# nullmax-vision/SimPB

Measured on AMD Instinct MI355X. Metric: frames/sec (6-cam sample) + MSDeformAttn HBM GB/s, R50 704x256 @1/2/4/8 GPU, higher is better.
Workload: dtype f32

## Files before the change

include/simpb_hip.h:

```cpp
#ifndef SIMPB_HIP_H
#define SIMPB_HIP_H

#ifdef __cplusplus
extern "C" {
#endif

#define SIMPB_OK 0
#define SIMPB_EINVAL 1
#define SIMPB_ELAUNCH 2

#define SIMPB_RECORD3D_WIDTH 15

int simpb_abi_version(void);

const char* simpb_last_error(void);

#define SIMPB_KERNEL_DAF 1
#define SIMPB_KERNEL_MSDA 2
int simpb_timing_enable(int capacity);
int simpb_timing_read(int kernel_id, float* ms_out, int max_n);
void simpb_timing_reset(void);

int simpb_deformable_aggregation_forward(
    float* output, const float* mc_ms_feat, const int* spatial_shape, const int* scale_start_index,
    const float* sample_location, const float* weights,
    int batch_size, int num_cams, int num_feat, int num_embeds, int num_scale,
    int num_anchors, int num_pts, int num_groups, void* stream);

int simpb_dfa_fused_forward(
    float* output, const void* mc_ms_feat, int feat_is_f16, const int* spatial_shape, const int* scale_start_index,
    const float* anchor, const float* learnable, const float* fix_scale, const float* projection_mat, const float* image_wh,
    const float* feat_logits, const float* cam_logits, float* loc_out, float* weights_out, int batch_size, int num_cams,
    int num_feat, int num_embeds, int num_scale, int num_anchors, int num_fix, int num_learn, int num_groups, void* stream);
int simpb_dfa_fused_forward_cams(
    float* output, const void* mc_ms_feat, int feat_is_f16, const int* spatial_shape, const int* scale_start_index,
    const float* anchor, const float* learnable, const float* fix_scale, const float* projection_mat, const float* image_wh,
    const float* feat_logits, const float* cam_logits, float* loc_out, float* weights_out, int batch_size, int num_cams,
    int num_feat, int num_embeds, int num_scale, int num_anchors, int num_fix, int num_learn, int num_groups,
    const unsigned char* cam_valid, void* stream);


int simpb_deformable_aggregation_backward(
    float* grad_mc_ms_feat, float* grad_sampling_location, float* grad_weights, const float* mc_ms_feat,
    const int* spatial_shape, const int* scale_start_index, const float* sample_location, const float* weights,
    const float* grad_output, int batch_size, int num_cams, int num_feat, int num_embeds, int num_scale,
    int num_anchors, int num_pts, int num_groups, void* stream);

int simpb_ms_deform_attn_grouped_forward(
    float* output, const float* value, const long long* spatial_shapes, const long long* level_start,
    const float* sampling_loc, const float* attn_weight, const int* query_cam,
    int batch_size, int num_cams, int num_value, int num_heads, int channels,
    int num_levels, int num_points, int num_query, void* stream);

int simpb_msda_linear_forward(float* agg, int ld_agg, const void* tokens, int tokens_are_f16,
                              const long long* spatial_shapes, const long long* level_start, const float* raw,
                              int ld_raw, const float* ref, int ld_ref, const int* query_cam, const int* m_live,
                              int batch_size, int num_cams, int num_value, int num_heads, int channels,
                              int num_levels, int num_points, int num_query, void* stream);

int simpb_ms_deform_attn_grouped_backward(
    float* grad_value, float* grad_sampling_loc, float* grad_attn_weight, const float* value,
    const long long* spatial_shapes, const long long* level_start, const float* sampling_loc, const float* attn_weight,
    const int* query_cam, const float* grad_output, int batch_size, int num_cams, int num_value, int num_heads,
    int channels, int num_levels, int num_points, int num_query, void* stream);

int simpb_linear_f32(float* y, const float* x, const float* weight, const float* bias, int M, int N, int K,
                     int relu, void* stream);

int simpb_linear_f16x3(float* y, const float* x, const void* weight_hi, const void* weight_lo, const float* bias, int M,
                       int N, int K, void* stream);

int simpb_linear_f16in_split(float* y, const void* x_f16, const void* weight_hi, const void* weight_lo, const float* bias,
                             int M, int N, int K, void* stream);

int simpb_stem_conv7x7_pool_f16(void* out, const void* img_nhwc4, const void* weight_packed, const void* bias,
                                int num_images, int height, int width, int out_channels, void* stream);

int simpb_image_to_nhwc4_f16(void* out, const float* img, long long stride_n, long long stride_c, long long stride_h,
                             long long stride_w, int num_images, int channels, int height, int width, void* stream);

#define SIMPB_PREPROCESS_MAX_TAPS 64
int simpb_preprocess_u8_nhwc4_f16(void* out, const void* src, void* mid, const int* kx, const int* xlo, const int* xn,
                                  const int* ky, const int* ylo, const int* yn, const void* lut, int num_images,
                                  int src_height, int src_width, int out_height, int out_width, int taps_x, int taps_y,
                                  int src_row0, int src_rows, int flip, int swap_rb, void* stream);

int simpb_preprocess_yuv420sp_nhwc4_f16(void* out, const void* src, void* mid, const int* kx, const int* xlo, const int* xn,
                                        const int* ky, const int* ylo, const int* yn, const void* lut, int num_images,
                                        int src_height, int src_width, int out_height, int out_width, int taps_x, int taps_y,
                                        int src_row0, int src_rows, int flip, int swap_rb, int vu_order, int yoff, int iy,
                                        int irv, int igu, int igv, int ibu, void* stream);

#define SIMPB_SURFACE_BGR 0
#define SIMPB_SURFACE_NV12 1
#define SIMPB_SURFACE_NV21 2
#define SIMPB_SURFACE_P010 3
int simpb_preprocess_surface_nhwc4_f16(void* out, const void* src, const void* image_table, void* mid, const int* kx,
                                       const int* xlo, const int* xn, const int* ky, const int* ylo, const int* yn,
                                       const void* lut, int num_images, int src_height, int src_width, int out_height,
                                       int out_width, int taps_x, int taps_y, int src_row0, int src_rows, int flip, int swap_rb,
                                       int format, long long pitch, long long chroma_pitch, long long chroma_offset,
                                       long long image_stride, int yoff, int iy, int irv, int igu, int igv, int ibu,
                                       void* stream);

int simpb_preprocess_mid_pitch(int out_width);

#define SIMPB_GEMM_MAX_SEGS 4
#define SIMPB_GEMM_MAX_JOBS 4
#define SIMPB_GEMM_OUT_F32 0
#define SIMPB_GEMM_OUT_SPLIT_HALFS 1
typedef struct simpb_gemm_job {
  const float* x[SIMPB_GEMM_MAX_SEGS];
  int ldx[SIMPB_GEMM_MAX_SEGS];
  int kseg[SIMPB_GEMM_MAX_SEGS];
  int num_seg;
  int M, N, K;
  const float* w;
  const float* bias;
  float* y;
  const int* m_live;
  int ldw, ldy, relu;
  int out_fmt;
  const int* row_flag;
  const float* bias2;
  const void* w_hi;
  const void* w_lo;
} simpb_gemm_job;
typedef struct simpb_gemm_args {
  int num_jobs;
  int reserved;
  simpb_gemm_job job[SIMPB_GEMM_MAX_JOBS];
} simpb_gemm_args;
int simpb_gemm_f32(const simpb_gemm_args* args, void* stream);

int simpb_layernorm_f32(float* out, int ldo, const float* x0, int ld0, int k0, const float* x1, int ld1, int k1,
                        const float* gamma, const float* beta, int num_rows, const int* m_live, void* stream);

#define SIMPB_MAX_LEVELS 8
int simpb_format_tokens(float* col_feats, const void* const* level_ptrs, const void* const* level_bias,
                        const int* level_hw, int num_levels, int num_images, int channels, int src_is_half, void* stream);

int simpb_bias_act_nhwc_f16(void* y, const void* bias, const void* residual, long long num_pixels, int channels,
                            int relu, void* stream);

int simpb_bias_relu_maxpool_nhwc_f16(void* y, const void* x, const void* bias, int num_images, int in_h, int in_w,
                                     int channels, void* stream);

int simpb_conv1x1_nhwc_f16(void* y, const void* x, const void* weight, const void* bias, const void* residual,
                           int num_images, int in_h, int in_w, int in_channels, int out_channels, int stride, int relu,
                           int residual_upsample2x, const void* input_bias, int variant, void* stream);

int simpb_conv3x3_nhwc_f16(void* y, float* tokens, void* tokens_f16, int tokens_per_cam, int level_start, const void* x,
                           const void* weight, const void* bias, int num_images, int in_h, int in_w, int in_channels,
                           int out_channels, int stride, int relu, int variant, void* stream);

int simpb_conv3x3_choose_variant(long long p_out, int in_channels, int out_channels);

int simpb_conv3x3_group_tokens_f16(int num_levels, float* tokens, void* tokens_f16, int tokens_per_cam, const int* level_start,
                                   const void* const* x, const void* const* weight, const void* const* bias, int num_images,
                                   const int* in_h, const int* in_w, int in_channels, int out_channels, int relu, void* stream);

int simpb_attention_f32(float* out, const float* q, const float* k, const float* v, const int* query_cam,
                        const int* group_start, int batch_size, int num_heads, int head_dim, int num_query,
                        int num_key, int ldq, int ldk, int ldv, int ldo, float scale, void* stream);

int simpb_attention_f32_split(float* out, const float* q, const float* k, const float* v, const int* query_cam,
                              const int* group_start, int batch_size, int num_heads, int head_dim, int num_query,
                              int num_key, int ldq, int ldk, int ldv, int ldo, float scale, void* stream);

int simpb_attention_split_halfs(float* out, const void* q, const void* k, const void* v, const int* query_cam,
                                const int* group_start, int batch_size, int num_heads, int head_dim, int num_query,
                                int num_key, int ldq, int ldk, int ldv, int ldo, void* stream);

#define SIMPB_MLP_MAX_OPS 12
#define SIMPB_MLP_MAX_CHAINS 8
#define SIMPB_MLP_POST_NONE 0
#define SIMPB_MLP_POST_REFINE3D 1
#define SIMPB_MLP_POST_REFINE2D 2
#define SIMPB_MLP_POST_SIGMOID 3
#define SIMPB_MLP_LINEAR 0
#define SIMPB_MLP_LAYERNORM 1
#define SIMPB_MLP_IN_ROWS 0
#define SIMPB_MLP_IN_SINE2D 1
#define SIMPB_MLP_IN_ROWS_LN 2
typedef struct simpb_mlp_op {
  int type, in_dim, out_dim, relu;
  const float* w;
  const float* b;
} simpb_mlp_op;
typedef struct simpb_mlp_chain {
  const float* x;
  const float* x2;
  float* out;
  const float* out_scale;
  int ldx, ldx2, ldo, in_dim, in_mode, n_ops;
  int post, ldres, res_cols, div_rows, div_col0, reserved;
  const float* res;
  const float* div;
  simpb_mlp_op ops[SIMPB_MLP_MAX_OPS];
  const float* ln_w;
  const float* ln_b;
  float* ln_out;
  int ld_ln_out, reserved2;
} simpb_mlp_chain;
typedef struct simpb_mlp_args {
  int num_rows, num_chains;
  int weights_transposed;
  int reserved;
  simpb_mlp_chain chain[SIMPB_MLP_MAX_CHAINS];
  const int* m_live;
} simpb_mlp_args;
int simpb_mlp_chain_forward(const simpb_mlp_args* args, void* stream);

int simpb_bank_get(float* anchor_out, unsigned char* mask_out, float* time_interval_out, const float* cached_anchor,
                   const float* T_temp2cur, const float* time_interval, int batch_size, int num_temp,
                   float max_time_interval, float default_time_interval, void* stream);
int simpb_bank_update(float* feature_out, float* anchor_out, long long* instance_id, int* index_scratch,
                      const float* feature, const float* anchor, const float* cls, const float* cached_feature,
                      const float* cached_anchor, const unsigned char* mask, int batch_size, int num_anchors,
                      int num_classes, int num_temp, int embed_dims, void* stream);
int simpb_bank_update_rank(int* index_scratch, const float* cls, int batch_size, int num_anchors, int num_classes,
                           int num_temp, void* stream);
int simpb_bank_update_merge(float* feature_out, float* anchor_out, float* embed_out, long long* instance_id, const int* index,
                            const float* feature, const float* anchor, const float* embed, const float* cached_feature,
                            const float* cached_anchor, const float* cached_embed, const unsigned char* mask, const int* hold,
                            int num_hold, const int* sticky, int batch_size, int num_anchors, int num_temp, int embed_dims,
                            int pos_embed_dims, void* stream);
int simpb_bank_cache(float* confidence, float* cached_feature, float* cached_anchor, long long* instance_id,
                     long long* prev_id, long long* ids_out, int* index_scratch, const float* feature, const float* anchor,
                     const float* cls, int batch_size, int num_anchors, int num_classes, int num_temp, int embed_dims,
                     int has_previous, float confidence_decay, int has_threshold, float threshold, const int* hold,
                     int num_hold, int* sticky, void* stream);
int simpb_bank_cache_streams(float* confidence, float* cached_feature, float* cached_anchor, long long* instance_id,
                             long long* prev_id, long long* ids_out, int* index_scratch, const float* feature, const float* anchor,
                             const float* cls, int batch_size, int num_anchors, int num_classes, int num_temp, int embed_dims,
                             int has_previous, float confidence_decay, int has_threshold, float threshold, const int* hold,
                             int num_hold, int* sticky, unsigned* sync_words, void* stream);

int simpb_bank_update_merge_active(float* feature_out, float* anchor_out, float* embed_out, long long* instance_id,
                                   const int* index, const float* feature, const float* anchor, const float* embed,
                                   const float* cached_feature, const float* cached_anchor, const float* cached_embed,
                                   const unsigned char* mask, const int* hold, int num_hold, const int* sticky, int batch_size,
                                   int num_anchors, int num_temp, int embed_dims, int pos_embed_dims,
                                   const unsigned char* active, void* stream);
int simpb_bank_cache_streams_active(float* confidence, float* cached_feature, float* cached_anchor, long long* instance_id,
                                    long long* prev_id, long long* ids_out, int* index_scratch, const float* feature,
                                    const float* anchor, const float* cls, int batch_size, int num_anchors, int num_classes,
                                    int num_temp, int embed_dims, int has_previous, float confidence_decay, int has_threshold,
                                    float threshold, const int* hold, int num_hold, int* sticky, unsigned* sync_words,
                                    const unsigned char* active, void* stream);

int simpb_decode3d_record(float* rec3d, int* rank_of_anchor, const float* cls, const float* quality, const float* box,
                          const long long* instance_id, int batch_size, int num_anchors, int num_classes,
                          int num_output, void* stream);
int simpb_decode2d_record(float* rec2d, const float* cls2d, const float* box2d, const int* q2a, const int* query_cam,
                          const int* rank_of_anchor, int batch_size, int num_query2d, int num_classes, int num_anchors,
                          float crop_w, float crop_h, float crop_y0, float resize, void* stream);

int simpb_decode2d_record_ragged(float* rec2d, const float* cls2d, const float* box2d, const int* q2a, const int* query_cam,
                                 const int* group_start, const int* rank_of_anchor, int batch_size, int rows_per_stream,
                                 int num_cams, int num_classes, int num_anchors, float crop_w, float crop_h, float crop_y0,
                                 float resize, void* stream);

int simpb_record2d_compact(float* out, long long out_stride, const float* rec2d, long long in_stride, int batch_size, int rows_in,
                           int rows_out, void* stream);

#define SIMPB_WORLD_WIDTH 16
#define SIMPB_WORLD_MAX_CLASSES 32
typedef struct simpb_world_tables {
  float class_range[SIMPB_WORLD_MAX_CLASSES];
  unsigned char attr_moving[SIMPB_WORLD_MAX_CLASSES];
  unsigned char attr_still[SIMPB_WORLD_MAX_CLASSES];
  float threshold;
  int has_threshold;
  int num_output;
} simpb_world_tables;
int simpb_world_record(double* world, int* count, const float* rec3d, const double* pose, const unsigned char* active,
                       simpb_world_tables tables, int num_streams, void* stream);

int simpb_topk_rows(float* values, int* indices, const float* scores, int batch_size, int n, int k, void* stream);

int simpb_rowdot_sigmoid(float* out, const float* x, int ldx, const float* w, const float* b, int num_rows, int k,
                         const int* m_live, void* stream);

int simpb_anchor_projection(float* out, const float* anchor, const float* T_src2dst, const float* time_interval,
                            int batch_size, int num_anchors, void* stream);

int simpb_msda_prep(float* sampling_loc, float* attn_weight, const float* raw, int ldraw, const float* ref, int ldref,
                    const long long* spatial_shapes, int num_rows, int num_heads, int num_levels, int num_points,
                    const int* m_live, void* stream);

int simpb_dfa_points(float* loc, float* key_points, const float* anchor, const float* learnable,
                     const float* fix_scale, const float* projection_mat, const float* image_wh, int batch_size,
                     int num_anchors, int num_fix, int num_learn, int num_cams, void* stream);
int simpb_dfa_points_cams(float* loc, float* key_points, const float* anchor, const float* learnable,
                          const float* fix_scale, const float* projection_mat, const float* image_wh, int batch_size,
                          int num_anchors, int num_fix, int num_learn, int num_cams, const unsigned char* cam_valid,
                          void* stream);

int simpb_dfa_weights(float* weights, const float* feat_logits, const float* cam_logits, int batch_size,
                      int num_anchors, int num_cams, int num_levels, int num_pts, int num_groups, void* stream);
int simpb_dfa_weights_cams(float* weights, const float* feat_logits, const float* cam_logits, int batch_size,
                           int num_anchors, int num_cams, int num_levels, int num_pts, int num_groups,
// ... 67 lines not shown
```

simpb_amd/_lib.py:

```python
import ctypes
import os

from .build import LIB

_lib = None

_P = ctypes.c_void_p
_I = ctypes.c_int
_F = ctypes.c_float
_LL = ctypes.c_longlong


class WorldTables(ctypes.Structure):
    _fields_ = [("class_range", _F * 32), ("attr_moving", ctypes.c_ubyte * 32), ("attr_still", ctypes.c_ubyte * 32),
                ("threshold", _F), ("has_threshold", _I), ("num_output", _I)]


SIGNATURES = {
    "simpb_abi_version": ([], _I),
    "simpb_last_error": ([], ctypes.c_char_p),
    "simpb_timing_enable": ([_I], _I),
    "simpb_timing_read": ([_I, _P, _I], _I),
    "simpb_timing_reset": ([], None),
    "simpb_deformable_aggregation_forward": ([_P] * 6 + [_I] * 8 + [_P], _I),
    "simpb_dfa_fused_forward": ([_P, _P, _I] + [_P] * 11 + [_I] * 9 + [_P], _I),
    "simpb_dfa_fused_forward_cams": ([_P, _P, _I] + [_P] * 11 + [_I] * 9 + [_P, _P], _I),
    "simpb_deformable_aggregation_backward": ([_P] * 9 + [_I] * 8 + [_P], _I),
    "simpb_ms_deform_attn_grouped_forward": ([_P] * 7 + [_I] * 8 + [_P], _I),
    "simpb_msda_linear_forward": ([_P, _I, _P, _I, _P, _P, _P, _I, _P, _I, _P, _P] + [_I] * 8 + [_P], _I),
    "simpb_ms_deform_attn_grouped_backward": ([_P] * 10 + [_I] * 8 + [_P], _I),
    "simpb_linear_f32": ([_P] * 4 + [_I] * 4 + [_P], _I),
    "simpb_linear_f16x3": ([_P] * 5 + [_I] * 3 + [_P], _I),
    "simpb_gemm_f32": ([_P, _P], _I),
    "simpb_layernorm_f32": ([_P, _I, _P, _I, _I, _P, _I, _I, _P, _P, _I, _P, _P], _I),
    "simpb_bias_act_nhwc_f16": ([_P, _P, _P, ctypes.c_longlong, _I, _I, _P], _I),
    "simpb_bias_relu_maxpool_nhwc_f16": ([_P, _P, _P, _I, _I, _I, _I, _P], _I),
    "simpb_conv1x1_nhwc_f16": ([_P] * 5 + [_I] * 8 + [_P, _I, _P], _I),
    "simpb_conv3x3_nhwc_f16": ([_P, _P, _P, _I, _I, _P, _P, _P] + [_I] * 8 + [_P], _I),
    "simpb_conv3x3_choose_variant": ([_LL, _I, _I], _I),
    "simpb_conv3x3_group_tokens_f16": ([_I, _P, _P, _I, _P, _P, _P, _P, _I, _P, _P, _I, _I, _I, _P], _I),
    "simpb_stem_conv7x7_pool_f16": ([_P] * 4 + [_I] * 4 + [_P], _I),
    "simpb_image_to_nhwc4_f16": ([_P, _P] + [ctypes.c_longlong] * 4 + [_I] * 4 + [_P], _I),
    "simpb_preprocess_u8_nhwc4_f16": ([_P] * 10 + [_I] * 11 + [_P], _I),
    "simpb_preprocess_yuv420sp_nhwc4_f16": ([_P] * 10 + [_I] * 18 + [_P], _I),
    "simpb_preprocess_surface_nhwc4_f16": ([_P] * 11 + [_I] * 12 + [_LL] * 4 + [_I] * 6 + [_P], _I),
    "simpb_preprocess_mid_pitch": ([_I], _I),
    "simpb_linear_f16in_split": ([_P] * 5 + [_I] * 3 + [_P], _I),
    "simpb_format_tokens": ([_P, _P, _P, _P, _I, _I, _I, _I, _P], _I),
    "simpb_attention_f32": ([_P] * 6 + [_I] * 9 + [_F, _P], _I),
    "simpb_attention_f32_split": ([_P] * 6 + [_I] * 9 + [_F, _P], _I),
    "simpb_attention_split_halfs": ([_P] * 6 + [_I] * 9 + [_P], _I),
    "simpb_mlp_chain_forward": ([_P, _P], _I),
    "simpb_bank_get": ([_P] * 6 + [_I] * 2 + [_F] * 2 + [_P], _I),
    "simpb_bank_update": ([_P] * 10 + [_I] * 5 + [_P], _I),
    "simpb_bank_update_rank": ([_P, _P] + [_I] * 4 + [_P], _I),
    "simpb_bank_update_merge": ([_P] * 13 + [_I, _P] + [_I] * 5 + [_P], _I),
    "simpb_bank_update_merge_active": ([_P] * 13 + [_I, _P] + [_I] * 5 + [_P, _P], _I),
    "simpb_bank_cache": ([_P] * 10 + [_I] * 6 + [_F, _I, _F, _P, _I, _P, _P], _I),
    "simpb_bank_cache_streams": ([_P] * 10 + [_I] * 6 + [_F, _I, _F, _P, _I, _P, _P, _P], _I),
    "simpb_bank_cache_streams_active": ([_P] * 10 + [_I] * 6 + [_F, _I, _F, _P, _I, _P, _P, _P, _P], _I),
    "simpb_decode3d_record": ([_P] * 6 + [_I] * 4 + [_P], _I),
    "simpb_decode2d_record": ([_P] * 6 + [_I] * 4 + [_F] * 4 + [_P], _I),
    "simpb_record2d_compact": ([_P, _LL, _P, _LL, _I, _I, _I, _P], _I),
    "simpb_decode2d_record_ragged": ([_P] * 7 + [_I] * 5 + [_F] * 4 + [_P], _I),
    "simpb_world_record": ([_P] * 5 + [WorldTables, _I, _P], _I),
    "simpb_topk_rows": ([_P, _P, _P, _I, _I, _I, _P], _I),
    "simpb_rowdot_sigmoid": ([_P, _P, _I, _P, _P, _I, _I, _P, _P], _I),
    "simpb_anchor_projection": ([_P] * 4 + [_I] * 2 + [_P], _I),
    "simpb_msda_prep": ([_P, _P, _P, _I, _P, _I, _P, _I, _I, _I, _I, _P, _P], _I),
    "simpb_dfa_points": ([_P] * 7 + [_I] * 5 + [_P], _I),
    "simpb_dfa_weights": ([_P] * 3 + [_I] * 6 + [_P], _I),
    "simpb_dfa_points_cams": ([_P] * 7 + [_I] * 5 + [_P, _P], _I),
    "simpb_dfa_weights_cams": ([_P] * 3 + [_I] * 6 + [_P, _P], _I),
    "simpb_alloc_project_cams": ([_P] * 5 + [_I] * 3 + [_F] * 5 + [_P, _P], _I),
    "simpb_alloc_project": ([_P] * 5 + [_I] * 3 + [_F] * 5 + [_P], _I),
    "simpb_alloc_compact": ([_P] * 3 + [_I] * 3 + [_P], _I),
    "simpb_alloc_group_start": ([_P] * 3 + [_I] * 3 + [_P], _I),
    "simpb_alloc_scatter": ([_P] * 12 + [_I] * 4 + [_F] * 2 + [_P], _I),
    "simpb_alloc_static": ([_P] * 15 + [_I] * 4 + [_F] * 5 + [_P], _I),
    "simpb_alloc_ragged": ([_P] * 15 + [_I] * 4 + [_F] * 5 + [_P], _I),
    "simpb_alloc_ragged_active": ([_P] * 15 + [_I] * 4 + [_F] * 5 + [_P, _P], _I),
    "simpb_alloc_static_cams": ([_P] * 15 + [_I] * 4 + [_F] * 5 + [_P, _P], _I),
    "simpb_alloc_ragged_cams": ([_P] * 15 + [_I] * 4 + [_F] * 5 + [_P, _P, _P], _I),
    "simpb_gather_rows": ([_P] * 3 + [_I] * 4 + [_P], _I),
    "simpb_aggregate_2d_to_3d": ([_P] * 8 + [_I] * 5 + [_P], _I),
    "simpb_aggregate_2d_to_3d_alpha": ([_P] * 9 + [_I, _I, _P, _P] + [_I] * 5 + [_P], _I),
}

ERRORS = {1: "SIMPB_EINVAL (bad pointer/size/layout)", 2: "SIMPB_ELAUNCH (kernel launch failed)"}


def lib():
    global _lib
    if _lib is None:
        if not os.path.exists(LIB):
            raise RuntimeError(
                f"{LIB} is missing: build it with `python -m simpb_amd.build` (hipcc --offload-arch=gfx950). "
                "simpb_amd has no fallback path for its HIP kernels.")
        import torch
        handle = ctypes.CDLL(LIB)
        for name, (argtypes, restype) in SIGNATURES.items():
            fn = getattr(handle, name)
            fn.argtypes = argtypes
            fn.restype = restype
        _lib = handle
    return _lib


def check(status, what):
    if status != 0:
        detail = ""
        if status == 2:
            detail = " - " + (lib().simpb_last_error() or b"").decode()
        raise RuntimeError(f"{what} failed: {ERRORS.get(status, status)}{detail}")
```

simpb_amd/csrc/conv1x1.hip:

```cpp
#include <hip/hip_runtime.h>
#include <hip/hip_fp16.h>
#include <type_traits>
#include "../../include/simpb_hip.h"
#include "mfma_f16.h"

extern "C" int simpb_check_launch(void);
extern "C" int simpb_conv_pointwise_staged(void* y, const void* x, const void* weight, const void* bias, const void* residual,
                                           int p_out, int in_h, int in_w, int ho, int wo, int in_channels, int out_channels,
                                           int stride, int relu, int residual_upsample2x, int tiling, void* stream);

namespace {

using f32x16 = __attribute__((ext_vector_type(16))) float;
using h16x8 = __attribute__((ext_vector_type(8))) _Float16;

constexpr int BM = 128, BN = 64, BK = 64;
constexpr int LDH = BK + 8;
constexpr int LDC = BN + 1;
constexpr int kThreads = 256;

__device__ __forceinline__ int up2(int p, int Ho, int Wo) {
  const int n = p / (Ho * Wo), rem = p - n * (Ho * Wo);
  const int ho = rem / Wo, wo = rem - ho * Wo;
  return (n * (Ho >> 1) + (ho >> 1)) * (Wo >> 1) + (wo >> 1);
}

__global__ __launch_bounds__(kThreads) void conv1x1_f16_kernel(_Float16* __restrict__ y, const _Float16* __restrict__ x,
                                                               const _Float16* __restrict__ w, const _Float16* __restrict__ bias,
                                                               const _Float16* __restrict__ residual, int P_out, int Cin,
                                                               int Cout, int relu, int stride, int Ho, int Wo, int H, int W,
                                                               int res_up, const _Float16* __restrict__ in_bias) {
  constexpr int kStageBytes = (BM + BN) * LDH * 2, kTileBytes = BM * LDC * 4;
  __shared__ __attribute__((aligned(16))) unsigned char smem[kStageBytes > kTileBytes ? kStageBytes : kTileBytes];
  _Float16* s_a = reinterpret_cast<_Float16*>(smem);
  _Float16* s_b = s_a + BM * LDH;
  float* s_c = reinterpret_cast<float*>(smem);
  const int tid = threadIdx.x;
  const int lane = tid & 63, wave = tid >> 6;
  const int r32 = lane & 31, kb = lane >> 5;
  const int p0 = blockIdx.x * BM, c0 = blockIdx.y * BN;

  constexpr int C8 = BK / 8, RS = kThreads / C8, NA = BM / RS, NB = BN / RS;
  const int sr = tid / C8, sc = (tid % C8) * 8;
  size_t arow[NA], brow[NB];
#pragma unroll
  for (int i = 0; i < NA; ++i) {
    int p = min(p0 + sr + RS * i, P_out - 1);
    if (stride != 1) {
      const int n = p / (Ho * Wo), rem = p - n * (Ho * Wo);
      const int ho = rem / Wo, wo = rem - ho * Wo;
      p = (n * H + ho * stride) * W + wo * stride;
    }
    arow[i] = (size_t)p * Cin + sc;
  }
#pragma unroll
  for (int i = 0; i < NB; ++i) brow[i] = (size_t)min(c0 + sr + RS * i, Cout - 1) * Cin + sc;
  const int nchunks = Cin / BK;
  h16x8 pa[2][NA], pb[2][NB], pin[2];
  auto fetch = [&](auto set_c, int chunk) __attribute__((always_inline)) {
    constexpr int set = decltype(set_c)::value;
    const int k0 = min(chunk, nchunks - 1) * BK;
    if (in_bias) pin[set] = *reinterpret_cast<const h16x8*>(in_bias + k0 + sc);
#pragma unroll
    for (int i = 0; i < NA; ++i) pa[set][i] = *reinterpret_cast<const h16x8*>(x + arow[i] + k0);
#pragma unroll
    for (int i = 0; i < NB; ++i) pb[set][i] = *reinterpret_cast<const h16x8*>(w + brow[i] + k0);
  };
  auto stash = [&](auto set_c, int) __attribute__((always_inline)) {
    constexpr int set = decltype(set_c)::value;
#pragma unroll
    for (int i = 0; i < NA; ++i) {
      h16x8 v = pa[set][i];
      if (in_bias) {
#pragma unroll
        for (int e = 0; e < 8; ++e) v[e] = (_Float16)fmaxf((float)v[e] + (float)pin[set][e], 0.f);
      }
      *reinterpret_cast<h16x8*>(&s_a[(sr + RS * i) * LDH + sc]) = v;
    }
#pragma unroll
    for (int i = 0; i < NB; ++i) *reinterpret_cast<h16x8*>(&s_b[(sr + RS * i) * LDH + sc]) = pb[set][i];
  };

  f32x16 acc[2];
#pragma unroll
  for (int n = 0; n < 2; ++n)
#pragma unroll
    for (int r = 0; r < 16; ++r) acc[n][r] = 0.f;

  auto multiply = [&]() __attribute__((always_inline)) {
#pragma unroll
    for (int ks = 0; ks < BK / 16; ++ks) {
      const h16x8 a = *reinterpret_cast<const h16x8*>(&s_a[(wave * 32 + r32) * LDH + 16 * ks + 8 * kb]);
#pragma unroll
      for (int n = 0; n < 2; ++n) {
        const h16x8 b = *reinterpret_cast<const h16x8*>(&s_b[(n * 32 + r32) * LDH + 16 * ks + 8 * kb]);
        acc[n] = simpb::mfma_32x32x16_f16(a, b, acc[n]);
      }
    }
  };

  const bool full = c0 + BN <= Cout;
  h16x8 rres[4];
  if (residual && full) {
#pragma unroll
    for (int i = 0; i < 4; ++i) {
      const int idx = tid + i * kThreads;
      int p = min(p0 + (idx >> 3), P_out - 1);
      if (res_up) p = up2(p, Ho, Wo);
      rres[i] = *reinterpret_cast<const h16x8*>(residual + (size_t)p * Cout + c0 + (idx & 7) * 8);
    }
  }

  fetch(std::integral_constant<int, 0>{}, 0);
  fetch(std::integral_constant<int, 1>{}, 1);
  for (int c = 0; c < nchunks; c += 2) {
    __syncthreads();
    stash(std::integral_constant<int, 0>{}, c);
    __syncthreads();
    fetch(std::integral_constant<int, 0>{}, c + 2);
    multiply();
    if (c + 1 < nchunks) {
      __syncthreads();
      stash(std::integral_constant<int, 1>{}, c + 1);
      __syncthreads();
      fetch(std::integral_constant<int, 1>{}, c + 3);
      multiply();
    }
  }

  __syncthreads();
#pragma unroll
  for (int n = 0; n < 2; ++n)
#pragma unroll
    for (int r = 0; r < 16; ++r) s_c[(wave * 32 + (r & 3) + 8 * (r >> 2) + 4 * kb) * LDC + n * 32 + r32] = acc[n][r];
  __syncthreads();
#pragma unroll
  for (int i = 0; i < 4; ++i) {
    const int idx = tid + i * kThreads;
    const int r = idx >> 3, c8 = (idx & 7) * 8;
    const int p = p0 + r;
    if (p >= P_out) continue;
    float v[8];
#pragma unroll
    for (int e = 0; e < 8; ++e) v[e] = s_c[r * LDC + c8 + e];
    if (full) {
      const h16x8 bv = *reinterpret_cast<const h16x8*>(bias + c0 + c8);
#pragma unroll
      for (int e = 0; e < 8; ++e) v[e] += (float)bv[e];
      if (residual) {
        const h16x8 rv = rres[i];
#pragma unroll
        for (int e = 0; e < 8; ++e) v[e] += (float)rv[e];
      }
      h16x8 o;
#pragma unroll
      for (int e = 0; e < 8; ++e) o[e] = (_Float16)(relu ? fmaxf(v[e], 0.f) : v[e]);
      *reinterpret_cast<h16x8*>(y + (size_t)p * Cout + c0 + c8) = o;
    } else {
#pragma unroll
      for (int e = 0; e < 8; ++e) {
        const int c = c0 + c8 + e;
        if (c < Cout) {
          float t = v[e] + (float)bias[c];
          if (residual) t += (float)residual[(size_t)(res_up ? up2(p, Ho, Wo) : p) * Cout + c];
          y[(size_t)p * Cout + c] = (_Float16)(relu ? fmaxf(t, 0.f) : t);
        }
      }
    }
  }
}

}

extern "C" int simpb_conv1x1_nhwc_f16(void* y, const void* x, const void* weight, const void* bias, const void* residual,
                                      int num_images, int in_h, int in_w, int in_channels, int out_channels, int stride,
                                      int relu, int residual_upsample2x, const void* input_bias, int variant, void* stream) {
  if (variant < 0 || variant > 4 || (input_bias && variant > 1)) return SIMPB_EINVAL;
  if (!y || !x || !weight || !bias || num_images <= 0 || in_h <= 0 || in_w <= 0 || in_channels <= 0 || out_channels <= 0 ||
      (stride != 1 && stride != 2) || in_channels % BK != 0 || out_channels % 8 != 0)
    return SIMPB_EINVAL;
  if ((reinterpret_cast<size_t>(y) | reinterpret_cast<size_t>(x) | reinterpret_cast<size_t>(weight) |
       reinterpret_cast<size_t>(bias) | reinterpret_cast<size_t>(residual) | reinterpret_cast<size_t>(input_bias)) & 15)
    return SIMPB_EINVAL;
  const int ho = (in_h - 1) / stride + 1, wo = (in_w - 1) / stride + 1;
  if (residual_upsample2x && (!residual || (ho & 1) || (wo & 1))) return SIMPB_EINVAL;
  const long long p_out = (long long)num_images * ho * wo;
  if (p_out > (1ll << 30)) return SIMPB_EINVAL;
  (void)hipGetLastError();
  if (variant == 0) {
    variant = (input_bias || in_channels < 512) ? 1 : 2;
    if (variant == 2 && in_channels >= 1024) {
      const long long t128 = ((p_out + 127) / 128) * ((out_channels + 63) / 64);
      if (t128 < 320) variant = 4;
    }
  }
  if (variant > 1) {
    if ((long long)num_images * in_h * in_w * in_channels > (1ll << 31) - 1) return SIMPB_EINVAL;
    return simpb_conv_pointwise_staged(y, x, weight, bias, residual, (int)p_out, in_h, in_w, ho, wo, in_channels, out_channels,
                                       stride, relu, residual_upsample2x, variant - 2, stream);
  }
  dim3 grid((unsigned)((p_out + BM - 1) / BM), (out_channels + BN - 1) / BN);
  if (grid.y > 65535) return SIMPB_EINVAL;
  hipLaunchKernelGGL(conv1x1_f16_kernel, grid, dim3(kThreads), 0, static_cast<hipStream_t>(stream),
                     static_cast<_Float16*>(y), static_cast<const _Float16*>(x), static_cast<const _Float16*>(weight),
                     static_cast<const _Float16*>(bias), static_cast<const _Float16*>(residual), (int)p_out, in_channels,
                     out_channels, relu, stride, ho, wo, in_h, in_w, residual_upsample2x ? 1 : 0,
                     static_cast<const _Float16*>(input_bias));
  return simpb_check_launch();
}
```

simpb_amd/plugin/ops.py:

```python
import ctypes

import torch
from torch.autograd.function import Function

from .. import _lib


def _ptr(t):
    return ctypes.c_void_p(t.data_ptr())


def _stream():
    return ctypes.c_void_p(torch.cuda.current_stream().cuda_stream)


def _require_gpu(*tensors):
    for t in tensors:
        if not t.is_cuda:
            raise RuntimeError("simpb_amd operators run on the GPU only (got a CPU tensor); "
                               "there is no CPU fallback")


_layout_ok = {}

# ... 260 lines not shown
    _lib.check(status, "simpb_msda_linear_forward")
    return agg


def linear_f32(x, weight, bias=None, relu=False):
    _require_gpu(x, weight)
    k = x.shape[-1]
    n = weight.shape[0]
    if weight.shape[1] != k or k % 32 != 0:
        raise ValueError(f"linear_f32 needs weight [N, K] with K % 32 == 0, got x {tuple(x.shape)} w {tuple(weight.shape)}")
    x2 = x.reshape(-1, k)
    if not x2.is_contiguous():
        x2 = x2.contiguous()
    x2, weight = x2.float(), weight.contiguous().float()
    if bias is not None:
        bias = bias.contiguous().float()
        if bias.numel() != n:
            raise ValueError("bias must have N elements")
    m = x2.shape[0]
    y = torch.empty(m, n, device=x.device, dtype=torch.float32)
    if m:
        status = _lib.lib().simpb_linear_f32(_ptr(y), _ptr(x2), _ptr(weight), _ptr(bias) if bias is not None else None,
                                             m, n, k, 1 if relu else 0, _stream())
        _lib.check(status, "simpb_linear_f32")
    return y.reshape(x.shape[:-1] + (n,))


def attention_f32(q, k, v, num_heads, query_cam=None, group_start=None, split=None):
    _require_gpu(q, k, v)
    bs, nq, e = q.shape
    nk = k.shape[1]
    hd = e // num_heads
    if hd != 64 or e != num_heads * 64 or k.shape[2] != e or v.shape[2] != e or v.shape[1] != nk:
        raise ValueError("attention_f32 needs head_dim 64 and matching q/k/v widths")

    def rows(t, n):
        if t.dtype != torch.float32:
            t = t.float()
        if t.stride(2) != 1 or (bs > 1 and t.stride(0) != n * t.stride(1)) or t.stride(1) % 4 or t.data_ptr() % 16:
            t = t.contiguous()
        return t, t.stride(1)

    q, ldq = rows(q, nq)
    k, ldk = rows(k, nk)
    v, ldv = rows(v, nk)
    out = torch.empty(bs, nq, e, device=q.device, dtype=torch.float32)
    if (query_cam is None) != (group_start is None):
        raise ValueError("query_cam and group_start go together")
    if query_cam is not None:
        if nk != nq or query_cam.dtype != torch.int32 or group_start.dtype != torch.int32 or query_cam.numel() != nq:
            raise ValueError("grouped attention needs i32 query_cam [N] / group_start [cams+1] over one slot set")
    if nq == 0:
        return out
    from . import routes
    mode = (1 if routes.R.attention_split_fp16 else 0) if split is None else int(split)
    tables = (_ptr(query_cam) if query_cam is not None else None, _ptr(group_start) if group_start is not None else None)
    if mode == 2:
        status = _lib.lib().simpb_attention_split_halfs(_ptr(out), _ptr(q), _ptr(k), _ptr(v), *tables, bs, num_heads, hd, nq, nk,
                                                        ldq, ldk, ldv, e, _stream())
    else:
        entry = _lib.lib().simpb_attention_f32_split if mode else _lib.lib().simpb_attention_f32
        status = entry(_ptr(out), _ptr(q), _ptr(k), _ptr(v), *tables, bs, num_heads, hd, nq, nk, ldq, ldk, ldv, e,
                       1.0 / (hd ** 0.5), _stream())
    _lib.check(status, "simpb_attention_f32")
    return out


def format_tokens(levels, bs, num_cams, biases=None):
    _require_gpu(*levels)
    c = levels[0].shape[1]
    dtype = levels[0].dtype
    shapes = tuple(tuple(f.shape[-2:]) for f in levels)
    srcs = []
    for f in levels:
        if f.shape[0] != bs * num_cams or f.shape[1] != c or f.dtype != dtype:
            raise ValueError("levels must share batch, channels and dtype")
        if not f.is_contiguous(memory_format=torch.channels_last):
            f = f.contiguous(memory_format=torch.channels_last)
        srcs.append(f)
    if dtype not in (torch.float16, torch.float32) or c % 8:
        raise ValueError("format_tokens takes f16/f32 levels with channels % 8 == 0")
    tokens = sum(h * w for h, w in shapes)
    col = torch.empty(bs, num_cams * tokens, c, device=levels[0].device, dtype=torch.float32)
    ptrs = (ctypes.c_void_p * len(srcs))(*[f.data_ptr() for f in srcs])
    hws = (ctypes.c_int * len(srcs))(*[h * w for h, w in shapes])
    bptrs = None
    if biases is not None:
        if len(biases) != len(srcs) or any(b is not None and (b.dtype != dtype or b.numel() != c or not b.is_contiguous()) for b in biases):
            raise ValueError("biases: one contiguous [C] tensor of the levels' dtype per level (or None)")
        bptrs = (ctypes.c_void_p * len(srcs))(*[b.data_ptr() if b is not None else None for b in biases])
    status = _lib.lib().simpb_format_tokens(_ptr(col), ptrs, bptrs, hws, len(srcs), bs * num_cams, c,
                                            1 if dtype == torch.float16 else 0, _stream())
    _lib.check(status, "simpb_format_tokens")
    spatial_shape, scale_start_index = _shape_tables(shapes, num_cams, col.device)
    return [col, spatial_shape, scale_start_index]


def bias_act_(y, bias, residual=None, relu=True):
    _require_gpu(y, bias)
    n, c, h, w = y.shape
    if (y.dtype != torch.float16 or not y.is_contiguous(memory_format=torch.channels_last) or bias.dtype != torch.float16
            or bias.numel() != c or c % 8):
        raise ValueError("bias_act_ takes a channels_last f16 tensor and an f16 bias with channels % 8 == 0")
    if residual is not None and (residual.shape != y.shape or residual.dtype != torch.float16
                                 or not residual.is_contiguous(memory_format=torch.channels_last)):
        raise ValueError("residual must match y (channels_last f16)")
    status = _lib.lib().simpb_bias_act_nhwc_f16(_ptr(y), _ptr(bias), _ptr(residual) if residual is not None else None,
                                                n * h * w, c, 1 if relu else 0, _stream())
    _lib.check(status, "simpb_bias_act_nhwc_f16")
    return y


def bias_relu_maxpool(x, bias):
    _require_gpu(x, bias)
    n, c, h, w = x.shape
    if (x.dtype != torch.float16 or not x.is_contiguous(memory_format=torch.channels_last) or bias.dtype != torch.float16
            or bias.numel() != c or c % 8 or not bias.is_contiguous()):
        raise ValueError("bias_relu_maxpool takes a channels_last f16 tensor and an f16 bias with channels % 8 == 0")
    y = torch.empty((n, c, (h - 1) // 2 + 1, (w - 1) // 2 + 1), device=x.device, dtype=torch.float16,
                    memory_format=torch.channels_last)
    _lib.check(_lib.lib().simpb_bias_relu_maxpool_nhwc_f16(_ptr(y), _ptr(x), _ptr(bias), n, h, w, c, _stream()),
               "simpb_bias_relu_maxpool_nhwc_f16")
    return y


def conv1x1_nhwc(x, weight, bias, residual=None, relu=True, stride=1, residual_upsample2x=False, input_bias=None, variant=0):
    _require_gpu(x, weight, bias)
    n, cin, h, w = x.shape
    cout = weight.shape[0]
    if (x.dtype != torch.float16 or not x.is_contiguous(memory_format=torch.channels_last) or weight.dtype != torch.float16
            or bias.dtype != torch.float16 or weight.numel() != cout * cin or cin % 64 or cout % 8 or stride not in (1, 2)):
        raise ValueError("conv1x1_nhwc takes channels_last f16 input, f16 [Cout, Cin, 1, 1] weight, Cin % 64 == 0, Cout % 8 == 0")
    ho, wo = (h - 1) // stride + 1, (w - 1) // stride + 1
    y = torch.empty((n, cout, ho, wo), device=x.device, dtype=torch.float16, memory_format=torch.channels_last)
    want = y.shape if not residual_upsample2x else (n, cout, ho // 2, wo // 2)
    if residual_upsample2x and (residual is None or ho % 2 or wo % 2):
        raise ValueError("residual_upsample2x needs a residual and even output sizes")
    if residual is not None and (tuple(residual.shape) != tuple(want) or residual.dtype != torch.float16
                                 or not residual.is_contiguous(memory_format=torch.channels_last)):
        raise ValueError("residual must match the output (channels_last f16)")
    if input_bias is not None and (input_bias.dtype != torch.float16 or input_bias.numel() != cin or not input_bias.is_contiguous()):
        raise ValueError("input_bias must be a contiguous f16 [Cin] tensor")
    w2 = weight.reshape(cout, cin)
    if not w2.is_contiguous():
        w2 = w2.contiguous()
    status = _lib.lib().simpb_conv1x1_nhwc_f16(_ptr(y), _ptr(x), _ptr(w2), _ptr(bias), _ptr(residual) if residual is not None else None,
                                               n, h, w, cin, cout, stride, 1 if relu else 0,
                                               1 if residual_upsample2x else 0,
                                               _ptr(input_bias) if input_bias is not None else None, variant, _stream())
    _lib.check(status, "simpb_conv1x1_nhwc_f16")
    return y


def conv3x3_nhwc(x, weight, bias, relu=True, stride=1, tokens=None, variant=0):
    _require_gpu(x, weight, bias)
    n, cin, h, w = x.shape
    cout = weight.shape[0]
    if (x.dtype != torch.float16 or not x.is_contiguous(memory_format=torch.channels_last) or weight.dtype != torch.float16
            or bias.dtype != torch.float16 or tuple(weight.shape) != (cout, cin, 3, 3) or cin % 64 or cout % 8
            or stride not in (1, 2) or bias.numel() != cout or not bias.is_contiguous()):
        raise ValueError("conv3x3_nhwc takes channels_last f16 input, f16 [Cout, Cin, 3, 3] weight, Cin % 64 == 0, Cout % 8 == 0")
    if not weight.is_contiguous(memory_format=torch.channels_last):
        weight = weight.contiguous(memory_format=torch.channels_last)
    ho, wo = (h - 1) // stride + 1, (w - 1) // stride + 1
    col16 = None
    if tokens is None:
        y = torch.empty((n, cout, ho, wo), device=x.device, dtype=torch.float16, memory_format=torch.channels_last)
        col, per_cam, start = None, 0, 0
    else:
        col, per_cam, start = tokens[:3]
        col16 = tokens[3] if len(tokens) > 3 else None
        y = None
        if col is None and col16 is None:
            raise ValueError("tokens: an f32 or an f16 token buffer")
        if col16 is not None and (col16.dtype != torch.float16 or not col16.is_contiguous()
                                  or (col is not None and col16.shape != col.shape)):
            raise ValueError("tokens: the f16 buffer must match col_feats")
        rows = col if col is not None else col16
        if ((col is not None and col.dtype != torch.float32) or not rows.is_contiguous() or rows.shape[-1] != cout
                or rows.numel() != n * per_cam * cout or start < 0 or start + ho * wo > per_cam):
            raise ValueError("tokens: (contiguous f32 [bs, cams * tokens_per_cam, Cout] with bs * cams == N, tokens_per_cam, level_start)")
    status = _lib.lib().simpb_conv3x3_nhwc_f16(_ptr(y) if y is not None else None, _ptr(col) if col is not None else None,
                                               _ptr(col16) if col16 is not None else None, per_cam, start, _ptr(x), _ptr(weight), _ptr(bias), n, h, w, cin, cout, stride,
                                               1 if relu else 0, variant, _stream())
    _lib.check(status, "simpb_conv3x3_nhwc_f16")
    return y


def conv3x3_variant_for(p_out, in_channels, out_channels):
    return int(_lib.lib().simpb_conv3x3_choose_variant(int(p_out), int(in_channels), int(out_channels)))


def conv3x3_group_tokens(xs, weights, biases, col, per_cam, starts, col16=None, relu=False):
    import ctypes
    if col is None and col16 is None:
        raise ValueError("conv3x3_group_tokens: an f32 or an f16 token buffer")
    rows = col if col is not None else col16
    _require_gpu(*xs, *weights, *biases, rows)
    n, cin = xs[0].shape[:2]
    cout = weights[0].shape[0]
    k = len(xs)
    if not (1 <= k <= 4 and len(weights) == k and len(biases) == k and len(starts) == k):
        raise ValueError("conv3x3_group_tokens: 1..4 levels, one weight / bias / start each")
    ws = []
    for x, w, b in zip(xs, weights, biases):
        if (x.dtype != torch.float16 or not x.is_contiguous(memory_format=torch.channels_last) or x.shape[0] != n or x.shape[1] != cin
                or w.dtype != torch.float16 or tuple(w.shape) != (cout, cin, 3, 3) or b.dtype != torch.float16 or b.numel() != cout
                or not b.is_contiguous() or cin % 64 or cout % 8):
            raise ValueError("conv3x3_group_tokens takes channels_last f16 inputs of one channel count, f16 [Cout, Cin, 3, 3] weights")
        ws.append(w if w.is_contiguous(memory_format=torch.channels_last) else w.contiguous(memory_format=torch.channels_last))
    if ((col is not None and col.dtype != torch.float32) or not rows.is_contiguous() or rows.shape[-1] != cout
            or rows.numel() != n * per_cam * cout
            or (col16 is not None and (col16.dtype != torch.float16 or not col16.is_contiguous() or col16.shape != rows.shape))):
        raise ValueError("conv3x3_group_tokens: col = contiguous f32 [bs, cams * tokens_per_cam, Cout] with bs * cams == N")
    arr_p, arr_i = ctypes.c_void_p * k, ctypes.c_int * k
    status = _lib.lib().simpb_conv3x3_group_tokens_f16(
        k, _ptr(col) if col is not None else None, _ptr(col16) if col16 is not None else None, int(per_cam), arr_i(*[int(v) for v in starts]),
        arr_p(*[x.data_ptr() for x in xs]), arr_p(*[w.data_ptr() for w in ws]), arr_p(*[b.data_ptr() for b in biases]), n,
        arr_i(*[x.shape[2] for x in xs]), arr_i(*[x.shape[3] for x in xs]), cin, cout, 1 if relu else 0, _stream())
    _lib.check(status, "simpb_conv3x3_group_tokens_f16")


def _stem_weight_packed(weight):
    tag = (weight.data_ptr(), weight._version, str(weight.device))
    hit = getattr(weight, "_simpb_stem_pack", None)
    if hit is None or hit[0] != tag:
        with torch.no_grad():
            w = weight.detach().float()
            full = torch.zeros(64, 4, 7, 8, device=w.device)
            full[:, :3, :, :7] = w
            pack = full.reshape(64, 4, 7, 4, 2).permute(2, 3, 4, 0, 1).contiguous().half()
        hit = (tag, pack)
        weight._simpb_stem_pack = hit
    return hit[1]


def stem_conv_pool(img, weight, bias):
    _require_gpu(img, weight, bias)
    n, c, h, w = img.shape
    if img.dtype != torch.float32 or c != 3 or tuple(weight.shape) != (64, 3, 7, 7) or bias.numel() != 64 or h < 1 or w < 1:
        raise ValueError("stem_conv_pool: f32 [N, 3, H, W] image, [64, 3, 7, 7] weight, 64 biases")
    lib = _lib.lib()
    x4 = torch.empty(n, h, w, 4, device=img.device, dtype=torch.float16)
    _lib.check(lib.simpb_image_to_nhwc4_f16(_ptr(x4), _ptr(img), img.stride(0), img.stride(1), img.stride(2), img.stride(3), n, c, h, w,
                                            _stream()), "simpb_image_to_nhwc4_f16")
    return stem_conv_pool_nhwc4(x4, weight, bias)


def stem_conv_pool_nhwc4(x4, weight, bias):
    _require_gpu(x4, weight, bias)
    if (x4.dtype != torch.float16 or x4.dim() != 4 or x4.shape[3] != 4 or not x4.is_contiguous() or tuple(weight.shape) != (64, 3, 7, 7)
            or bias.numel() != 64 or x4.shape[1] < 1 or x4.shape[2] < 1):
        raise ValueError("stem_conv_pool_nhwc4: contiguous f16 [N, H, W, 4] image, [64, 3, 7, 7] weight, 64 biases")
    n, h, w, _ = x4.shape
    lib = _lib.lib()
    ho, wo = (h - 1) // 2 + 1, (w - 1) // 2 + 1
    hp, wp = (ho - 1) // 2 + 1, (wo - 1) // 2 + 1
    out = torch.empty((n, 64, hp, wp), device=x4.device, dtype=torch.float16, memory_format=torch.channels_last)
    b16 = bias if bias.dtype == torch.float16 and bias.is_contiguous() else bias.half().contiguous()
    _lib.check(lib.simpb_stem_conv7x7_pool_f16(_ptr(out), _ptr(x4), _ptr(_stem_weight_packed(weight)), _ptr(b16), n, h, w, 64,
                                               _stream()), "simpb_stem_conv7x7_pool_f16")
    return out


def preprocess_frames(frames, plan, out=None):
    return plan.run(frames, out=out)


def topk_rows(scores, k):
    _require_gpu(scores)
    if scores.dim() != 2 or scores.shape[1] > 2048:
        raise ValueError("topk_rows takes [bs, n <= 2048] scores")
    scores = scores.contiguous().float()
    bs, n = scores.shape
    values = torch.empty(bs, k, device=scores.device, dtype=torch.float32)
    index = torch.empty(bs, k, device=scores.device, dtype=torch.int32)
    if bs and k:
        _lib.check(_lib.lib().simpb_topk_rows(_ptr(values), _ptr(index), _ptr(scores), bs, n, k, _stream()),
                   "simpb_topk_rows")
    return values, index.long()




def linear_split(x, weight, bias=None):
    _require_gpu(x, weight)
    k = x.shape[-1]
    if weight.shape[1] != k or k % 32:
        raise ValueError("linear_split: x [..., K], weight [N, K], K a multiple of 32")
    tag = (weight.data_ptr(), weight._version, str(weight.device))
    hit = getattr(weight, "_simpb_split_lin", None)
    if hit is None or hit[0] != tag:
        from .dense import split_in_window
        if torch.cuda.is_current_stream_capturing() or not split_in_window(weight):
            hit = (tag, None, None) if not torch.cuda.is_current_stream_capturing() else None
        else:
            with torch.no_grad():
                w = weight.detach().float()
                hi = w.half()
                lo = ((w - hi.float()) * 2048.0).half()
            hit = (tag, hi.contiguous(), lo.contiguous())
        if hit is not None:
            weight._simpb_split_lin = hit
    if hit is None or hit[1] is None:
        return linear_f32(x.float() if x.dtype == torch.float16 else x, weight, bias)
    m, n = x.numel() // k, weight.shape[0]
# ... 14 lines not shown
```

Baseline: 448.8.

## Add column-walking conv1x1 kernel that keeps the input tile resident across output blocks

Adds a new 1x1 conv kernel family that loads a pixel tile of the whole input (Cin up to 256) into LDS once, then walks several output-channel blocks. It double-buffers weights and prefetches residual and bias for each block. The default variant chooser now uses a table of shapes that match this backbone's layers and routes them to the new variants. The goal is to stop re-reading the input activations for every output-channel tile and to raise MFMA utilisation, at the cost of more LDS and register pressure and a shape-specific dispatch table.

```diff
diff --git a/include/simpb_hip.h b/include/simpb_hip.h
--- a/include/simpb_hip.h
+++ b/include/simpb_hip.h
@@ -149,6 +149,9 @@
 int simpb_conv1x1_nhwc_f16(void* y, const void* x, const void* weight, const void* bias, const void* residual,
                            int num_images, int in_h, int in_w, int in_channels, int out_channels, int stride, int relu,
                            int residual_upsample2x, const void* input_bias, int variant, void* stream);
+
+int simpb_conv1x1_choose_variant(long long p_out, int in_channels, int out_channels, int stride, int has_residual,
+                                 int has_input_bias);
 
 int simpb_conv3x3_nhwc_f16(void* y, float* tokens, void* tokens_f16, int tokens_per_cam, int level_start, const void* x,
                            const void* weight, const void* bias, int num_images, int in_h, int in_w, int in_channels,
diff --git a/simpb_amd/_lib.py b/simpb_amd/_lib.py
--- a/simpb_amd/_lib.py
+++ b/simpb_amd/_lib.py
@@ -36,6 +36,7 @@
     "simpb_bias_act_nhwc_f16": ([_P, _P, _P, ctypes.c_longlong, _I, _I, _P], _I),
     "simpb_bias_relu_maxpool_nhwc_f16": ([_P, _P, _P, _I, _I, _I, _I, _P], _I),
     "simpb_conv1x1_nhwc_f16": ([_P] * 5 + [_I] * 8 + [_P, _I, _P], _I),
+    "simpb_conv1x1_choose_variant": ([_LL] + [_I] * 5, _I),
     "simpb_conv3x3_nhwc_f16": ([_P, _P, _P, _I, _I, _P, _P, _P] + [_I] * 8 + [_P], _I),
     "simpb_conv3x3_choose_variant": ([_LL, _I, _I], _I),
     "simpb_conv3x3_group_tokens_f16": ([_I, _P, _P, _I, _P, _P, _P, _P, _I, _P, _P, _I, _I, _I, _P], _I),
diff --git a/simpb_amd/csrc/conv1x1.hip b/simpb_amd/csrc/conv1x1.hip
--- a/simpb_amd/csrc/conv1x1.hip
+++ b/simpb_amd/csrc/conv1x1.hip
@@ -170,12 +170,258 @@
   }
 }
 
+__device__ __forceinline__ void wave_lds_order() {
+  __builtin_amdgcn_fence(__ATOMIC_RELEASE, "wavefront");
+  __builtin_amdgcn_wave_barrier();
+  __builtin_amdgcn_fence(__ATOMIC_ACQUIRE, "wavefront");
+}
+
+template <int BM_, int NCH, int NB_>
+__global__ __launch_bounds__(kThreads) void conv1x1_colwalk_kernel(_Float16* __restrict__ y, const _Float16* __restrict__ x,
+                                                                   const _Float16* __restrict__ w, const _Float16* __restrict__ bias,
+                                                                   const _Float16* __restrict__ residual, int P_out, int Cout,
+                                                                   int relu, int stride, int Ho, int Wo, int H, int W, int res_up,
+                                                                   const _Float16* __restrict__ in_bias) {
+  static_assert(BM_ == 128 || BM_ == 64, "wave -> tile maps exist for 128 and 64 pixels");
+  constexpr int Cin = NCH * BK, LDX = Cin + 8;
+  constexpr int WBUF = NCH == 1 ? 2 : 1;
+  constexpr int kXBytes = BM_ * LDX * 2, kWBytes = WBUF * BN * LDX * 2, kCBytes = 32 * LDC * 4;
+  static_assert(kXBytes + kWBytes + kCBytes <= 160 * 1024, "LDS of one CU");
+  __shared__ __attribute__((aligned(16))) unsigned char smem[kXBytes + kWBytes + kCBytes];
+  _Float16* s_x = reinterpret_cast<_Float16*>(smem);
+  _Float16* s_w = reinterpret_cast<_Float16*>(smem + kXBytes);
+  float* s_c = reinterpret_cast<float*>(smem + kXBytes + kWBytes);
+  const int tid = threadIdx.x;
+  const int lane = tid & 63, wave = tid >> 6;
+  const int r32 = lane & 31, kb = lane >> 5;
+  const int p0 = blockIdx.x * BM_;
+  const int nblk = (Cout + BN - 1) / BN, j0 = blockIdx.y * NB_;
+  const int nj = min(NB_, nblk - j0);
+  constexpr int NT = BM_ == 128 ? 2 : 1;
+  const int rowb = BM_ == 128 ? 32 * wave : 32 * (wave & 1);
+  const int colb = BM_ == 128 ? 0 : 32 * (wave >> 1);
+  constexpr int PW = 4 * NT, RP = 64 / PW, NI = 32 / RP;
+  const int er = rowb + lane / PW, ec = colb + (lane % PW) * 8;
+  const int tb = rowb * RP / 32;
+
+  constexpr int RS = kThreads / (BK / 8), NA = BM_ / RS, NW = BN / RS;
+  const int sr = tid / (BK / 8), sc = (tid % (BK / 8)) * 8;
+  h16x8 pw[NCH][NW];
+  auto fetch_w = [&](int c0) __attribute__((always_inline)) {
+#pragma unroll
+    for (int i = 0; i < NW; ++i) {
+      const _Float16* row = w + (size_t)min(c0 + sr + RS * i, Cout - 1) * Cin + sc;
+#pragma unroll
+      for (int c = 0; c < NCH; ++c) pw[c][i] = *reinterpret_cast<const h16x8*>(row + c * BK);
+    }
+  };
+  auto stash_w = [&](_Float16* sw) __attribute__((always_inline)) {
+#pragma unroll
+    for (int i = 0; i < NW; ++i)
+#pragma unroll
+      for (int c = 0; c < NCH; ++c) *reinterpret_cast<h16x8*>(&sw[(sr + RS * i) * LDX + c * BK + sc]) = pw[c][i];
+  };
+  constexpr int RD = BM_ == 64 ? (NB_ < 4 ? NB_ : 4) : (NB_ < 2 ? NB_ : 2);
+  size_t rrow[NI];
+  h16x8 rres[RD][NI], rcur[NI], bnext, bcur;
+  if (residual) {
+#pragma unroll
+    for (int i = 0; i < NI; ++i) {
+      int p = min(p0 + er + RP * i, P_out - 1);
+      if (res_up) p = up2(p, Ho, Wo);
+      rrow[i] = (size_t)p * Cout;
+    }
+  }
+  auto fetch_res = [&](int slot, int c0) __attribute__((always_inline)) {
+    if (residual && c0 + BN <= Cout) {
+#pragma unroll
+      for (int i = 0; i < NI; ++i) rres[slot][i] = *reinterpret_cast<const h16x8*>(residual + rrow[i] + c0 + ec);
+    }
+  };
+  auto fetch_bias = [&](int c0) __attribute__((always_inline)) {
+    if (c0 + BN <= Cout) bnext = *reinterpret_cast<const h16x8*>(bias + c0 + ec);
+  };
+
+  {
+    h16x8 pa[NCH][NA];
+#pragma unroll
+    for (int i = 0; i < NA; ++i) {
+      int p = min(p0 + sr + RS * i, P_out - 1);
+      if (stride != 1) {
+        const int n = p / (Ho * Wo), rem = p - n * (Ho * Wo);
+        const int ho = rem / Wo, wo = rem - ho * Wo;
+        p = (n * H + ho * stride) * W + wo * stride;
+      }
+      const _Float16* row = x + (size_t)p * Cin + sc;
+#pragma unroll
+      for (int c = 0; c < NCH; ++c) pa[c][i] = *reinterpret_cast<const h16x8*>(row + c * BK);
+    }
+    fetch_w(j0 * BN);
+    fetch_bias(j0 * BN);
+#pragma unroll
+    for (int d = 0; d < RD; ++d)
+      if (d < nj) fetch_res(d, (j0 + d) * BN);
+#pragma unroll
+    for (int c = 0; c < NCH; ++c) {
+      h16x8 pin;
+      if (in_bias) pin = *reinterpret_cast<const h16x8*>(in_bias + c * BK + sc);
+#pragma unroll
+      for (int i = 0; i < NA; ++i) {
+        h16x8 v = pa[c][i];
+        if (in_bias) {
+#pragma unroll
+          for (int e = 0; e < 8; ++e) v[e] = (_Float16)fmaxf((float)v[e] + (float)pin[e], 0.f);
+        }
+        *reinterpret_cast<h16x8*>(&s_x[(sr + RS * i) * LDX + c * BK + sc]) = v;
+      }
+    }
+    stash_w(s_w);
+  }
+  __syncthreads();
+
+#pragma unroll
+  for (int j = 0; j < NB_; ++j) {
+    if (j >= nj) break;
+    const int c0 = (j0 + j) * BN;
+    const bool full = c0 + BN <= Cout, more = j + 1 < nj;
+    bcur = bnext;
+    if (residual) {
+#pragma unroll
+      for (int i = 0; i < NI; ++i) rcur[i] = rres[j % RD][i];
+    }
+    if (more) {
+      fetch_w(c0 + BN);
+      fetch_bias(c0 + BN);
+    }
+    if (j + RD < nj) fetch_res(j % RD, c0 + RD * BN);
+    const _Float16* sw = s_w + (j & (WBUF - 1)) * BN * LDX;
+    f32x16 acc[NT];
+#pragma unroll
+    for (int n = 0; n < NT; ++n)
+#pragma unroll
+      for (int r = 0; r < 16; ++r) acc[n][r] = 0.f;
+#pragma unroll
+    for (int c = 0; c < NCH; ++c)
+#pragma unroll
+      for (int ks = 0; ks < BK / 16; ++ks) {
+        const h16x8 a = *reinterpret_cast<const h16x8*>(&s_x[(rowb + r32) * LDX + c * BK + 16 * ks + 8 * kb]);
+#pragma unroll
+        for (int n = 0; n < NT; ++n) {
+          const h16x8 b = *reinterpret_cast<const h16x8*>(&sw[(colb + n * 32 + r32) * LDX + c * BK + 16 * ks + 8 * kb]);
+          acc[n] = simpb::mfma_32x32x16_f16(a, b, acc[n]);
+        }
+      }
+#pragma unroll
+    for (int i = 0; i < NI; ++i) {
+      wave_lds_order();
+#pragma unroll
+      for (int n = 0; n < NT; ++n)
+#pragma unroll
+        for (int r = i * RP / 2; r < (i + 1) * RP / 2; ++r)
+          s_c[(tb + (r & 3) + 8 * ((r >> 2) - i * RP / 8) + 4 * kb) * LDC + colb + n * 32 + r32] = acc[n][r];
+      wave_lds_order();
+      const int p = p0 + er + RP * i;
+      if (p >= P_out) continue;
+      float v[8];
+#pragma unroll
+      for (int e = 0; e < 8; ++e) v[e] = s_c[(tb + lane / PW) * LDC + ec + e];
+      if (full) {
+        const h16x8 bv = bcur;
+#pragma unroll
+        for (int e = 0; e < 8; ++e) v[e] += (float)bv[e];
+        if (residual) {
+          const h16x8 rv = rcur[i];
+#pragma unroll
+          for (int e = 0; e < 8; ++e) v[e] += (float)rv[e];
+        }
+        h16x8 o;
+#pragma unroll
+        for (int e = 0; e < 8; ++e) o[e] = (_Float16)(relu ? fmaxf(v[e], 0.f) : v[e]);
+        *reinterpret_cast<h16x8*>(y + (size_t)p * Cout + c0 + ec) = o;
+      } else {
+#pragma unroll
+        for (int e = 0; e < 8; ++e) {
+          const int c = c0 + ec + e;
+          if (c < Cout) {
+            float t = v[e] + (float)bias[c];
+            if (residual) t += (float)residual[rrow[i] + c];
+            y[(size_t)p * Cout + c] = (_Float16)(relu ? fmaxf(t, 0.f) : t);
+          }
+        }
+      }
+    }
+    if (more) {
+      if (WBUF == 1) __syncthreads();
+      stash_w(s_w + ((j + 1) & (WBUF - 1)) * BN * LDX);
+      __syncthreads();
+    }
+  }
+}
+
+constexpr int kColwalkFirst = 5, kColwalkLast = 10;
+
+template <int BM_, int NCH, int NB_>
+void launch_colwalk_as(hipStream_t stream, long long p_out, int out_channels, _Float16* y, const _Float16* x, const _Float16* w,
+                       const _Float16* bias, const _Float16* residual, int relu, int stride, int ho, int wo, int in_h, int in_w,
+                       int res_up, const _Float16* in_bias) {
+  const int nblk = (out_channels + BN - 1) / BN;
+  dim3 grid((unsigned)((p_out + BM_ - 1) / BM_), (nblk + NB_ - 1) / NB_);
+  hipLaunchKernelGGL((conv1x1_colwalk_kernel<BM_, NCH, NB_>), grid, dim3(kThreads), 0, stream, y, x, w, bias, residual, (int)p_out,
+                     out_channels, relu, stride, ho, wo, in_h, in_w, res_up, in_bias);
+}
+
+template <int BM_, int NB_, class... Args>
+int launch_colwalk_nch(int nch, Args... args) {
+  switch (nch) {
+    case 1: launch_colwalk_as<BM_, 1, NB_>(args...); return 0;
+    case 2: launch_colwalk_as<BM_, 2, NB_>(args...); return 0;
+    case 3: launch_colwalk_as<BM_, 3, NB_>(args...); return 0;
+    case 4: launch_colwalk_as<BM_, 4, NB_>(args...); return 0;
+  }
+  return SIMPB_EINVAL;
+}
+
+template <class... Args>
+int launch_colwalk(int variant, int nch, Args... args) {
+  switch (variant) {
+    case 5: return launch_colwalk_nch<128, 2>(nch, args...);
+    case 6: return launch_colwalk_nch<128, 4>(nch, args...);
+    case 7: return launch_colwalk_nch<64, 1>(nch, args...);
+    case 8: return launch_colwalk_nch<64, 2>(nch, args...);
+    case 9: return launch_colwalk_nch<64, 4>(nch, args...);
+    case 10: return launch_colwalk_nch<64, 8>(nch, args...);
+  }
+  return SIMPB_EINVAL;
+}
+
+}
+
+extern "C" int simpb_conv1x1_choose_variant(long long p_out, int in_channels, int out_channels, int stride, int has_residual,
+                                            int has_input_bias) {
+  int variant = (has_input_bias || in_channels < 512) ? 1 : 2;
+  if (variant == 1 && !has_input_bias) {
+    static const struct { int p_out, cin, cout, stride, residual, variant; } kMeasured[] = {
+        {67584, 64, 64, 1, 0, 7},   {67584, 64, 256, 1, 0, 7},  {67584, 64, 256, 1, 1, 7},
+        {67584, 256, 64, 1, 0, 7},  {67584, 256, 128, 1, 0, 10}, {16896, 256, 512, 2, 0, 8},
+        {16896, 128, 512, 1, 1, 7}, {4224, 256, 1024, 1, 1, 7}, {67584, 256, 256, 1, 1, 9}};
+    for (const auto& m : kMeasured)
+      if (p_out == m.p_out && in_channels == m.cin && out_channels == m.cout && stride == m.stride &&
+          (has_residual != 0) == (m.residual != 0))
+        return m.variant;
+  }
+  if (variant == 2 && in_channels >= 1024) {
+    const long long t128 = ((p_out + 127) / 128) * ((out_channels + 63) / 64);
+    if (t128 < 320) variant = 4;
+  }
+  return variant;
 }
 
 extern "C" int simpb_conv1x1_nhwc_f16(void* y, const void* x, const void* weight, const void* bias, const void* residual,
                                       int num_images, int in_h, int in_w, int in_channels, int out_channels, int stride,
                                       int relu, int residual_upsample2x, const void* input_bias, int variant, void* stream) {
-  if (variant < 0 || variant > 4 || (input_bias && variant > 1)) return SIMPB_EINVAL;
+  const bool colwalk = variant >= kColwalkFirst && variant <= kColwalkLast;
+  if (variant < 0 || variant > kColwalkLast || (input_bias && variant > 1 && !colwalk)) return SIMPB_EINVAL;
+  if (colwalk && in_channels > 4 * BK) return SIMPB_EINVAL;
   if (!y || !x || !weight || !bias || num_images <= 0 || in_h <= 0 || in_w <= 0 || in_channels <= 0 || out_channels <= 0 ||
       (stride != 1 && stride != 2) || in_channels % BK != 0 || out_channels % 8 != 0)
     return SIMPB_EINVAL;
@@ -187,12 +433,15 @@
   const long long p_out = (long long)num_images * ho * wo;
   if (p_out > (1ll << 30)) return SIMPB_EINVAL;
   (void)hipGetLastError();
-  if (variant == 0) {
-    variant = (input_bias || in_channels < 512) ? 1 : 2;
-    if (variant == 2 && in_channels >= 1024) {
-      const long long t128 = ((p_out + 127) / 128) * ((out_channels + 63) / 64);
-      if (t128 < 320) variant = 4;
-    }
+  if (variant == 0)
+    variant = simpb_conv1x1_choose_variant(p_out, in_channels, out_channels, stride, residual ? 1 : 0, input_bias ? 1 : 0);
+  if (variant >= kColwalkFirst) {
+    if ((out_channels + BN - 1) / BN > 65535) return SIMPB_EINVAL;
+    const int status = launch_colwalk(variant, in_channels / BK, static_cast<hipStream_t>(stream), p_out, out_channels,
+                                      static_cast<_Float16*>(y), static_cast<const _Float16*>(x), static_cast<const _Float16*>(weight),
+                                      static_cast<const _Float16*>(bias), static_cast<const _Float16*>(residual), relu, stride, ho, wo,
+                                      in_h, in_w, residual_upsample2x ? 1 : 0, static_cast<const _Float16*>(input_bias));
+    return status ? status : simpb_check_launch();
   }
   if (variant > 1) {
     if ((long long)num_images * in_h * in_w * in_channels > (1ll << 31) - 1) return SIMPB_EINVAL;
diff --git a/simpb_amd/plugin/ops.py b/simpb_amd/plugin/ops.py
--- a/simpb_amd/plugin/ops.py
+++ b/simpb_amd/plugin/ops.py
@@ -436,6 +436,11 @@
     return y
 
 
+def conv1x1_variant_for(p_out, in_channels, out_channels, stride=1, has_residual=False, has_input_bias=False):
+    return int(_lib.lib().simpb_conv1x1_choose_variant(int(p_out), int(in_channels), int(out_channels), int(stride),
+                                                       1 if has_residual else 0, 1 if has_input_bias else 0))
+
+
 def conv3x3_nhwc(x, weight, bias, relu=True, stride=1, tokens=None, variant=0):
     _require_gpu(x, weight, bias)
     n, cin, h, w = x.shape
```

Result: faster. 453.7 (median of 6 runs) (+1.1%).
